# Tongji-MIC-Lab/TDVC

Hardware: AMD Instinct MI355X
Metric: 1080p P-frames/sec (encode + reconstruct, lambda=2048 config) (higher is better)
Workload: dtype f16; 1 GPU; 1x 1920x1080 (padded 1088x1920) 7-frame synthetic GOP (seed 1234), batch 1, P-frames coded in GOP order; gop=7, batch=1, parallelism=gop-sharded x1, weights=closed-form filler (no checkpoint ships)

## Files before the change

### include/tdvc_hip.h

```cpp
#ifndef TDVC_HIP_H
#define TDVC_HIP_H

#include <stdint.h>

#ifdef __cplusplus
extern "C" {
#endif

#define TDVC_OK 0
#define TDVC_EINVAL (-1)
#define TDVC_ENOSUP (-2)

typedef struct {
  void* p;
  int32_t N, H, W, C;
  int64_t sn;
  int32_t sp;
  int32_t dtype;
} tdvc_fmap;

enum { TDVC_F16 = 0, TDVC_F32 = 1 };
enum { TDVC_ACT_NONE = 0, TDVC_ACT_RELU = 1, TDVC_ACT_LRELU = 2, TDVC_ACT_CLAMP01 = 3, TDVC_ACT_SIGMOID = 4 };
enum { TDVC_GDN_NONE = 0, TDVC_GDN_FWD = 1, TDVC_GDN_INV = 2 };
enum { TDVC_OUT_NHWC = 0,
// ... 56 lines not shown
  const float* bias;
  int32_t act1; float slope1;
  int32_t act2; float slope2;
  int32_t add_input;
  tdvc_fmap res2;
} tdvc_conv_pair_desc;
int64_t tdvc_conv_pair_packed_bytes(void);
int tdvc_pack_conv_pair_weights(const float* w1_oihw, const float* w2_oihw, uint16_t* dst);
int tdvc_conv_pair_supported(const tdvc_conv_pair_desc* d);
int tdvc_conv_pair(const tdvc_conv_pair_desc* d, void* stream);

typedef struct {
  tdvc_fmap s, a, y;
  int32_t nslices;
  int32_t slice_stride;
  const void* wt;
  const float* bias_t;
  const void* w3;
  const float* bias3;
  float slope;
} tdvc_lf_tail_desc;
int tdvc_lf_tail_supported(const tdvc_lf_tail_desc* d);
int tdvc_lf_tail(const tdvc_lf_tail_desc* d, void* stream);

typedef struct {
  tdvc_fmap x, om, y;
  const void* w;
  const float* bias;
  int32_t groups;
  int32_t act; float slope; int32_t round_before_act;
  void* x_planar;
} tdvc_dcn_desc;
int tdvc_dcn_fused(const tdvc_dcn_desc* d, void* stream);

int tdvc_dcn_v2_forward_f32(const float* input, const float* weight, const float* bias,
                            const float* offset, const float* mask, float* output,
                            int B, int C, int H, int W, int Cout,
                            int kh, int kw, int sh, int sw, int ph, int pw, int dh, int dw,
                            int deformable_group, void* stream);
int tdvc_dcn_v2_backward_f32(const float* input, const float* weight, const float* bias,
                             const float* offset, const float* mask, const float* grad_output,
                             float* grad_input, float* grad_offset, float* grad_mask,
                             float* grad_weight, float* grad_bias, float* columns,
                             int B, int C, int H, int W, int Cout,
                             int kh, int kw, int sh, int sw, int ph, int pw, int dh, int dw,
                             int deformable_group, void* stream);
// ... 220 lines not shown
```

### tdvc_amd/_lib.py

```python
from __future__ import annotations

import ctypes as C
import os

_HERE = os.path.dirname(os.path.abspath(__file__))
LIB_PATH = os.path.join(_HERE, "libtdvc_hip.so")

MAX_TAPS = 49
F16, F32 = 0, 1
ACT_NONE, ACT_RELU, ACT_LRELU, ACT_CLAMP01, ACT_SIGMOID = 0, 1, 2, 3, 4
GDN_NONE, GDN_FWD, GDN_INV = 0, 1, 2
OUT_NHWC, OUT_SHUFFLE2, OUT_NCHW_F32 = 0, 1, 2


class FMapDesc(C.Structure):
    _fields_ = [("p", C.c_void_p), ("N", C.c_int32), ("H", C.c_int32), ("W", C.c_int32), ("C", C.c_int32),
                ("sn", C.c_int64), ("sp", C.c_int32), ("dtype", C.c_int32)]


class ConvDesc(C.Structure):
    _fields_ = [("x", FMapDesc), ("y", FMapDesc), ("w", C.c_void_p), ("bias", C.c_void_p),
                ("cout", C.c_int32), ("ntaps", C.c_int32),
                ("tap_dy", C.c_int8 * MAX_TAPS), ("tap_dx", C.c_int8 * MAX_TAPS),
                ("kh", C.c_int32), ("kw", C.c_int32), ("stride", C.c_int32), ("pad", C.c_int32),
                ("ck", C.c_int32), ("square_input", C.c_int32), ("gdn", C.c_int32),
                ("aux", FMapDesc), ("act", C.c_int32), ("slope", C.c_float),
                ("round_before_act", C.c_int32), ("res", FMapDesc), ("res2", FMapDesc), ("out_mode", C.c_int32), ("s2d", C.c_int32),
                ("bcast_T", C.c_int32), ("bcast_slope", C.c_float), ("chan_sum", C.c_void_p), ("flow", FMapDesc)]


class DcnDesc(C.Structure):
    _fields_ = [("x", FMapDesc), ("om", FMapDesc), ("y", FMapDesc), ("w", C.c_void_p), ("bias", C.c_void_p),
                ("groups", C.c_int32), ("act", C.c_int32), ("slope", C.c_float), ("round_before_act", C.c_int32), ("x_planar", C.c_void_p)]


class ConvPairDesc(C.Structure):
    _fields_ = [("x", FMapDesc), ("y", FMapDesc), ("w", C.c_void_p), ("bias", C.c_void_p), ("act1", C.c_int32), ("slope1", C.c_float),
                ("act2", C.c_int32), ("slope2", C.c_float), ("add_input", C.c_int32), ("res2", FMapDesc)]


class LfTailDesc(C.Structure):
    _fields_ = [("s", FMapDesc), ("a", FMapDesc), ("y", FMapDesc), ("nslices", C.c_int32), ("slice_stride", C.c_int32),
                ("wt", C.c_void_p), ("bias_t", C.c_void_p), ("w3", C.c_void_p), ("bias3", C.c_void_p), ("slope", C.c_float)]


class WgradReduceJob(C.Structure):
    _fields_ = [("work", C.c_void_p), ("bwork", C.c_void_p), ("row_off", C.c_void_p), ("chan_off", C.c_void_p), ("tap_off", C.c_void_p),
                ("bias_index", C.c_void_p), ("dw", C.c_void_p), ("db", C.c_void_p), ("scale", C.c_float),
                ("nworkers", C.c_int32), ("cow", C.c_int32), ("ciw", C.c_int32), ("ntaps", C.c_int32), ("cout", C.c_int32), ("cin", C.c_int32),
                ("wblocks", C.c_int32), ("nblocks", C.c_int32)]


_P = C.c_void_p
_FM = C.POINTER(FMapDesc)


class CdfTablesDesc(C.Structure):
    _fields_ = [("cdfs", _P), ("sizes", _P), ("offsets", _P), ("stride", C.c_int32), ("ncdfs", C.c_int32)]


class CdfTablesDevDesc(C.Structure):
    _fields_ = [("cdf16", _P), ("starts", _P), ("sizes", _P), ("offsets", _P), ("n16", C.c_int32), ("ncdfs", C.c_int32)]


class ArLoopDesc(C.Structure):
    _fields_ = [("y_hat", FMapDesc), ("params", FMapDesc), ("x1", FMapDesc), ("pc", FMapDesc), ("gp", FMapDesc),
# ... 78 lines not shown
    "tdvc_ssim_level": (_i, [_P, _P, _i, _i, _i, _i, _P, _i, _f, _f, _P, _P, _P, _i64, _P]),
    "tdvc_avgpool2_pad_f32": (_i, [_P, _i64, _i, _i, _P, _P]),
    "tdvc_ssim_level_backward": (_i, [_P, _P, _i, _i, _i, _i, _P, _i, _f, _f, _P, _P, _f, _P, _P, _P]),
    "tdvc_msssim_level_grads": (_i, [_P, _P, _P, _i, _i, _P, _P, _P, _P, _P]),
    "tdvc_dcn_col2im_work_floats": (_i64, [_i, _i, _i, _i]),
    "tdvc_dcn_col2im_tile": (_i, []),
    "tdvc_dcn_col2im": (_i, [_FM, _FM, _FM, _i, _P, _FM, _P, _i64, _P]),
    "tdvc_dcn_col2im_det": (_i, [_FM, _FM, _FM, _i, _P, _FM, _P, _i64, _P, _P, _P, _i, _P]),
    "tdvc_dcn_far_apply": (_i, [_P, _P, _P, _i, _P, _P]),
    "tdvc_conv_wgrad_work_floats": (_i64, [_i] * 6),
    "tdvc_conv_wgrad": (_i, [_FM, _FM] + [_i] * 6 + [_P] * 5 + [_i, _f, _P, _P, _i64, _P]),
    "tdvc_conv_wgrad_bias": (_i, [_FM, _FM] + [_i] * 6 + [_P] * 5 + [_i, _f, _P, _P, _P, _P, _i64, _P]),
    "tdvc_conv_wgrad_partials": (_i, [_FM, _FM] + [_i] * 6 + [_P] * 5 + [_i, _f, _P, _P, _P, _P, _i64, C.POINTER(WgradReduceJob), _P]),
    "tdvc_wgrad_reduce_batch": (_i, [_P, _P, _i, _i, _P]),
    "tdvc_gdn_backward": (_i, [_FM, _FM, _FM, _i, _FM, _FM, _P]),
    "tdvc_mul2_accumulate": (_i, [_FM, _FM, _FM, _P]),
    "tdvc_dcn_fused": (_i, [C.POINTER(DcnDesc), _P]),
    "tdvc_conv_pair_packed_bytes": (_i64, []),
    "tdvc_pack_conv_pair_weights": (_i, [_P, _P, _P]),
    "tdvc_conv_pair_supported": (_i, [C.POINTER(ConvPairDesc)]),
    "tdvc_conv_pair": (_i, [C.POINTER(ConvPairDesc), _P]),
    "tdvc_lf_tail_supported": (_i, [C.POINTER(LfTailDesc)]),
    "tdvc_lf_tail": (_i, [C.POINTER(LfTailDesc), _P]),
    "tdvc_dcn_v2_forward_f32": (_i, [_P] * 6 + [_i] * 14 + [_P]),
    "tdvc_dcn_v2_backward_f32": (_i, [_P] * 12 + [_i] * 14 + [_P]),
    "tdvc_nchw_to_fmap": (_i, [_P, _i, _FM, _P]),
    "tdvc_fmap_to_nchw": (_i, [_FM, _i, _P, _P]),
    "tdvc_scale_act_res": (_i, [_FM, _P, _i, _f, _FM, _f, _FM, _FM, _P]),
    "tdvc_add_flow": (_i, [_FM, _FM, _P]),
    "tdvc_bcast_add_act": (_i, [_FM, _FM, _i, _f, _P]),
    "tdvc_channel_sum": (_i, [_FM, _P, _i, _P]),
    "tdvc_se_gate": (_i, [_P, _i, _f, _i, _i, _i, _P, _P, _P, _P, _P, _P]),
    "tdvc_upsample2x": (_i, [_FM, _FM, _P]),
    "tdvc_avgpool2": (_i, [_FM, _FM, _P]),
    "tdvc_spynet_level_input": (_i, [_FM, _FM, _FM, _FM, _FM, _P]),
    "tdvc_resize_bilinear": (_i, [_FM, _FM, _P, _P]),
    "tdvc_avgpool_k_work_floats": (_i64, [_i, _i, _i, _i, _i]),
    "tdvc_avgpool_k": (_i, [_FM, _i, _P, _i, _i, _P, _i64, _P]),
    "tdvc_patch_match": (_i, [_P, _P, _i, _i, _i, _i, _P, _P]),
    "tdvc_match_gather": (_i, [_FM, _FM, _P, _i, _i, _i, _FM, _P]),
    "tdvc_eb_forward": (_i, [_FM, _P, _FM, _FM, _P, _P, _i, _P]),
    "tdvc_gc_forward": (_i, [_FM, _FM, _FM, _P, _P, _i, _P]),
    "tdvc_quantize": (_i, [_FM, _FM, _FM, _P]),
    "tdvc_rans_encode": (_i64, [_P, _P, _i64, _P, C.c_int32, _P, _P, _P, _i64]),
    "tdvc_rans_decode": (_i, [_P, _i64, _P, _i64, _P, C.c_int32, _P, _P, _P]),
    "tdvc_rans_encode_lanes": (_i64, [_P, _P, _i64, _i, _i, _P, C.c_int32, _P, _P, _P, _i64]),
# ... 40 lines not shown
```

### tdvc_amd/csrc/conv_dispatch.hip

```cpp
#include <stdlib.h>

#include "conv_common.h"

using convk::ConvParams;
bool conv_v2_eligible(const tdvc_conv_desc* d, int Ho, int Wo); int launch_conv_v2(const ConvParams& p, int cout_blocks, int N, hipStream_t st);
bool conv_v3_eligible(const tdvc_conv_desc* d, int Ho, int Wo); int launch_conv_v3(const ConvParams& p, int cout_blocks, int N, hipStream_t st);
bool conv_v5_eligible(const tdvc_conv_desc* d, int Ho, int Wo); int launch_conv_v5(const ConvParams& p, int cout_blocks, int N, hipStream_t st); int conv_v5_chan_sum_rows(int Ho, int Wo, int cout_blocks, int N);
bool conv_v7_eligible(const tdvc_conv_desc* d, const ConvParams& p, int Ho, int Wo); int launch_conv_v7(const ConvParams& p, int cout_blocks, int N, hipStream_t st);
bool conv_v9_eligible(const tdvc_conv_desc* d, int Ho, int Wo, bool v3_ok); int launch_conv_v9(const ConvParams& p, int ck8, int cout_tiles32, int N, hipStream_t st);
bool conv_v10_eligible(const tdvc_conv_desc* d, const ConvParams& p, int Ho, int Wo); int launch_conv_v10(const ConvParams& p, int cout_blocks, int N, hipStream_t st);
bool conv_v11_eligible(const tdvc_conv_desc* d, const ConvParams& p, int Ho, int Wo); int launch_conv_v11(const ConvParams& p, int cout_blocks, int N, hipStream_t st);
int conv_row_geometry(const tdvc_conv_desc* d, const ConvParams& p, int Ho, int Wo); int launch_conv_row(int geo, const ConvParams& p, int N, hipStream_t st);
bool conv_c8_eligible(const tdvc_conv_desc* d, const ConvParams& p, int Ho, int Wo); int launch_conv_c8(const ConvParams& p, int N, hipStream_t st);
bool conv_n16_eligible(const tdvc_conv_desc* d, int Ho, int Wo); int launch_conv_n16(const ConvParams& p, int N, hipStream_t st);
bool gdn128_eligible(const tdvc_conv_desc* d, const ConvParams& p, int Ho, int Wo); int launch_gdn128(const ConvParams& p, int N, hipStream_t st);
int conv_direct_lds_bytes(const tdvc_conv_desc* d);
int conv_cout_tiles(int cout);
int launch_conv_direct(const ConvParams& p, int ck8, int stride, int N, hipStream_t st);
int conv_f32_validate(const tdvc_conv_desc* d, int& Ho, int& Wo);

namespace {
const char* const kSwitchEnv[convk::SW_COUNT] = {nullptr, "TDVC_CONV_NO_V3", "TDVC_CONV_NO_V5", "TDVC_CONV_NO_V7", "TDVC_CONV_NO_V9", "TDVC_CONV_NO_V10",
                                                 "TDVC_CONV_NO_V11", "TDVC_CONV_NO_ROW", "TDVC_CONV_NO_C8", "TDVC_CONV_NO_N16", "TDVC_CONV_NO_GDN128", "TDVC_CONV_NO_HEAD3"};
int g_enabled[convk::SW_COUNT] = {1, 1, 1, 1, 1, 1, 1, 15, 1, 1, 1, 1};
// ... 222 lines not shown
  ConvParams p;
  Pick k = {d, 0, 0, -1};
  if (const int rc = prepare(d, p, k.Ho, k.Wo)) return rc;
  p.reverse = query != LAUNCH ? 0 : next_walk_reverse();
  const Entry* e = select(k, p);
  const bool csum_ok = e && e->name == kNameV5 && k.cout_blocks() == 1 && p.simple == 2;
  if (query_rows) return csum_ok ? conv_v5_chan_sum_rows(k.Ho, k.Wo, 1, k.N()) : 0;
  if (query == QUERY_FLOW) return conv_flow_ok(d, e, p) && (!d->flow.p || flow_map_ok(d, k.Ho, k.Wo)) ? 1 : 0;
  TDVC_CHECK(!d->chan_sum || (csum_ok && (reinterpret_cast<uintptr_t>(d->chan_sum) & 15) == 0),
             "tdvc_conv2d: chan_sum on a conv whose kernel has no fused channel sum (tdvc_conv_chan_sum_rows() == 0) or unaligned");
  p.csum = d->chan_sum;
  if (!e) return TDVC_EINVAL;
  if (d->flow.p) {
    TDVC_CHECK(conv_flow_ok(d, e, p) && flow_map_ok(d, k.Ho, k.Wo), "%s", kFlowMsg);
    p.flow = to_dev(d->flow);
  }
  kernel_name(e, k, g_last_kernel);
  return e->launch(k, p, reinterpret_cast<hipStream_t>(stream));
}

}

void tdvc_conv_walk_advance(int launches) { g_walk_parity += (unsigned)launches; }

extern "C" void tdvc_debug_set_conv_walk(int mode) { g_walk_mode = mode; }
extern "C" int tdvc_conv2d(const tdvc_conv_desc* d, void* stream) { return conv2d_impl(d, stream, LAUNCH); }
extern "C" int tdvc_conv_chan_sum_rows(const tdvc_conv_desc* d) { return conv2d_impl(d, nullptr, QUERY_ROWS); }
extern "C" int tdvc_conv_flow_supported(const tdvc_conv_desc* d) { return conv2d_impl(d, nullptr, QUERY_FLOW); }
extern "C" const char* tdvc_last_conv_kernel(void) { return g_last_kernel; }

extern "C" const char* tdvc_conv_select(const tdvc_conv_desc* d) {
  static thread_local char name[48];
  if (!d) { tdvc_set_error("tdvc_conv_select: null descriptor"); return nullptr; }
  if (d->x.dtype == TDVC_F32) {
    int Ho, Wo;
    if (d->flow.p) { tdvc_set_error("%s", kFlowMsg); return nullptr; }
    return conv_f32_validate(d, Ho, Wo) == TDVC_OK ? "conv_f32" : nullptr;
  }
  ConvParams p;
  Pick k = {d, 0, 0, -1};
  if (prepare(d, p, k.Ho, k.Wo) != TDVC_OK) return nullptr;
  const Entry* e = select(k, p);
  if (!e) return nullptr;
  if (d->flow.p && !(conv_flow_ok(d, e, p) && flow_map_ok(d, k.Ho, k.Wo))) { tdvc_set_error("%s", kFlowMsg); return nullptr; }
  kernel_name(e, k, name);
  return name;
// ... 2 lines not shown
```

### tdvc_amd/csrc/lib.cpp

```cpp
#include <hip/hip_runtime.h>
#include <stdarg.h>
#include <stddef.h>
#include <stdio.h>

#include <mutex>

#include "../../include/tdvc_hip.h"

static thread_local char g_err[512] = "";

void tdvc_set_error(const char* fmt, ...) {
  va_list ap;
  va_start(ap, fmt);
  vsnprintf(g_err, sizeof(g_err), fmt, ap);
  va_end(ap);
}

static_assert(sizeof(tdvc_cdf_tables) == 32 && offsetof(tdvc_cdf_tables, ncdfs) == 28, "tdvc_cdf_tables layout");
static_assert(sizeof(tdvc_cdf_tables_dev) == 40 && offsetof(tdvc_cdf_tables_dev, ncdfs) == 36, "tdvc_cdf_tables_dev layout");
static_assert(sizeof(tdvc_ar_loop) == 272 && offsetof(tdvc_ar_loop, sym_dev) == 264, "tdvc_ar_loop layout");
static_assert(sizeof(tdvc_lf_tail_desc) == 168 && offsetof(tdvc_lf_tail_desc, slope) == 160, "tdvc_lf_tail_desc layout");
static_assert(sizeof(tdvc_lanes_enc) == 104 && offsetof(tdvc_lanes_enc, info) == 96, "tdvc_lanes_enc layout");

extern "C" int tdvc_abi_version(void) { return 16; }
extern "C" const char* tdvc_last_error(void) { return g_err; }

static thread_local const int* g_pred = nullptr;
static thread_local int g_pred_taken = 0, g_pred_last = 0;
static thread_local const int* g_pred_img = nullptr;
static thread_local int g_pred_img_n = 0;

extern "C" int tdvc_set_predicate(const int* flag) {
  if (reinterpret_cast<uintptr_t>(flag) & 3) { tdvc_set_error("tdvc_set_predicate: flag must be 4-byte aligned"); return TDVC_EINVAL; }
  if (flag && g_pred_img) { tdvc_set_error("tdvc_set_predicate: a per-image predicate is set (clear it first)"); return TDVC_EINVAL; }
  g_pred = flag;
  return TDVC_OK;
}
extern "C" int tdvc_set_predicate_images(const int* flags, int n) {
  if (!flags || n == 0) { g_pred_img = nullptr; g_pred_img_n = 0; return TDVC_OK; }
  if (reinterpret_cast<uintptr_t>(flags) & 3) { tdvc_set_error("tdvc_set_predicate_images: flags must be 4-byte aligned"); return TDVC_EINVAL; }
  if (n < 1 || n > TDVC_MAX_PREDICATE_IMAGES) { tdvc_set_error("tdvc_set_predicate_images: 1 <= n <= %d images, got %d", TDVC_MAX_PREDICATE_IMAGES, n); return TDVC_EINVAL; }
  if (g_pred) { tdvc_set_error("tdvc_set_predicate_images: a launch predicate is set (clear it first)"); return TDVC_EINVAL; }
  g_pred_img = flags; g_pred_img_n = n;
  return TDVC_OK;
}
const int* tdvc_launch_predicate_images(int N) {
  if (!g_pred_img || N != g_pred_img_n) return nullptr;
// ... 52 lines not shown
```

### tdvc_amd/csrc/pointwise.hip

```cpp
#include "pointwise_common.h"

namespace {

__global__ void nchw_to_fmap_kernel(const float* src, int C, FMap y) {
  const long npix = (long)y.H * y.W;
  const long i = (long)blockIdx.x * blockDim.x + threadIdx.x;
  if (i >= npix * y.N) return;
  const int n = (int)(i / npix);
  const long pix = i % npix;
  for (int c0 = 0; c0 < y.C; c0 += 8) {
    float v[8];
#pragma unroll
    for (int j = 0; j < 8; ++j) v[j] = (c0 + j < C) ? src[((long)n * C + c0 + j) * npix + pix] : 0.f;
    store8(y, n, pix, c0, v);
  }
}

__global__ void fmap_to_nchw_kernel(FMap x, int C, float* dst) {
  const long npix = (long)x.H * x.W;
  const long i = (long)blockIdx.x * blockDim.x + threadIdx.x;
  if (i >= npix * x.N) return;
  const int n = (int)(i / npix);
  const long pix = i % npix;
  for (int c0 = 0; c0 < C; c0 += 8) {
// ... 242 lines not shown
  if (tid < Cmid) {
    float s = b1[tid];
    for (int c = 0; c < C; ++c) s += w1[tid * C + c] * mean[c];
    mid[tid] = s > 0.f ? s : 0.f;
  }
  __syncthreads();
  if (tid < C) {
    float s = b2[tid];
    for (int j = 0; j < Cmid; ++j) s += w2[tid * Cmid + j] * mid[j];
    gate[(long)n * C + tid] = 1.f / (1.f + expf(-s));
  }
}

__global__ void upsample2x_kernel(FMap x, FMap y) {
  const int chunks = x.C / 8;
  const long npix = (long)y.H * y.W;
  const long i = (long)blockIdx.x * blockDim.x + threadIdx.x;
  if (i >= npix * chunks * y.N) return;
  const int c = (int)(i % chunks) * 8;
  const long t = i / chunks;
  const long pix = t % npix;
  const int n = (int)(t / npix);
  const int oy = (int)(pix / y.W), ox = (int)(pix % y.W);
  const float sy = fmaxf((oy + 0.5f) * 0.5f - 0.5f, 0.f), sx = fmaxf((ox + 0.5f) * 0.5f - 0.5f, 0.f);
  const int y0 = (int)sy, x0 = (int)sx;
  const int y1 = y0 + (y0 < x.H - 1), x1 = x0 + (x0 < x.W - 1);
  const float ly1 = sy - y0, lx1 = sx - x0, ly0 = 1.f - ly1, lx0 = 1.f - lx1;
  float a[8], b[8], cc[8], d[8], v[8];
  load8(x, n, (long)y0 * x.W + x0, c, a);
  load8(x, n, (long)y0 * x.W + x1, c, b);
  load8(x, n, (long)y1 * x.W + x0, c, cc);
  load8(x, n, (long)y1 * x.W + x1, c, d);
#pragma unroll
  for (int j = 0; j < 8; ++j) v[j] = ly0 * (lx0 * a[j] + lx1 * b[j]) + ly1 * (lx0 * cc[j] + lx1 * d[j]);
  store8(y, n, pix, c, v);
}

__global__ void avgpool2_kernel(FMap x, FMap y) {
  const long npix = (long)y.H * y.W;
  const long i = (long)blockIdx.x * blockDim.x + threadIdx.x;
  if (i >= npix * y.N) return;
  const int n = (int)(i / npix);
  const long pix = i % npix;
  const int oy = (int)(pix / y.W), ox = (int)(pix % y.W);
  const float* xp = reinterpret_cast<const float*>(x.p) + (long)n * x.sn;
  float* yp = reinterpret_cast<float*>(y.p) + (long)n * y.sn + pix * y.sp;
  const long p00 = ((long)(2 * oy) * x.W + 2 * ox) * x.sp, p10 = p00 + (long)x.W * x.sp;
  for (int c = 0; c < y.C; ++c)
    yp[c] = (xp[p00 + c] + xp[p00 + x.sp + c] + xp[p10 + c] + xp[p10 + x.sp + c]) * 0.25f;
}

struct PyramidMaps { FMap x[2]; FMap y[2][5]; };
template <bool VEC>
__global__ __launch_bounds__(256) void avgpool2_pyramid_kernel(const PyramidMaps a) {
  __shared__ __attribute__((aligned(16))) float lv[2][16 * 16 * 4];
  const int m = blockIdx.z & 1, n = blockIdx.z >> 1, tid = threadIdx.x;
  const int C = a.y[0][0].C;
// ... 691 lines not shown
```

### tdvc_amd/model/modules.py

```python
from __future__ import annotations

import torch
import torch.nn as nn

from .. import ops
from ..ops import ACT_LRELU, ACT_NONE, ACT_RELU, FM
from .ring import SlotRing


class PackCache:

    def _pk(self, key, fn):
        c = self.__dict__.setdefault("_packed", {})
        if key not in c:
            c[key] = fn()
        return c[key]


def _dev(m: nn.Module):
    return next(m.parameters()).device


def pk_conv(owner: PackCache, name: str, conv: nn.Module, **kw) -> ops.PackedConv:
    def build():
# ... 58 lines not shown
        if self.conv1.in_channels == 64 and ops.conv_pair_supported(x, out, res2) and (out is None or out.desc().p != x.desc().p):
            pp = self._pk("pair", lambda: ops.pack_conv_pair(self.conv1.weight, self.conv1.bias, self.conv2.weight, self.conv2.bias))
            return ops.conv_pair(x, pp, out=out, act1=ACT_RELU, act2=ACT_NONE, add_input=True, res2=res2)
        t = ops.conv(x, pk_conv(self, "c1", self.conv1), act=ACT_RELU)
        return ops.conv(t, pk_conv(self, "c2", self.conv2), out=out, res=x, res2=res2)


def res_stack(n, ch=64):
    return nn.Sequential(*[Res_Block(ch) for _ in range(n)])


def run_stack(stack, x: FM, out: FM | None = None, res2: FM | None = None) -> FM:
    n = len(stack)
    for i, blk in enumerate(stack):
        last = i == n - 1
        x = blk.run(x, out=out if last else None, res2=res2 if last else None)
    return x


PYRAMID_FUSED = True
FLOW_EPILOGUE = True
RESID_FUSED = True
RGB_HEAD = True


def glue_fusions_allowed(module: nn.Module, traced: bool = False) -> bool:
    return not module.training and ops.TAPE is None and ops.PROFILE is None and not traced


class SPyNetBasicModule(nn.Module):
    def __init__(self):
        super().__init__()
        ch = [8, 32, 64, 32, 16, 2]
        self.basic_module = nn.Sequential(*[ConvAct(ch[i], ch[i + 1], 7, 1, 3) for i in range(5)])


class SPyNet(nn.Module, PackCache):

    def __init__(self):
        super().__init__()
        self.basic_module = nn.ModuleList([SPyNetBasicModule() for _ in range(6)])
        self.register_buffer("mean", torch.tensor([0.485, 0.456, 0.406]).view(1, 3, 1, 1))
        self.register_buffer("std", torch.tensor([0.229, 0.224, 0.225]).view(1, 3, 1, 1))

    def compute_flow(self, ref: FM, supp: FM, fused: bool = False, f32: bool = False) -> FM:
        if fused and PYRAMID_FUSED and ops.avgpool2_pyramid_supported(ref, supp):
# ... 83 lines not shown
            t = ops.conv(cat2.ch(64 * k, 64), pk_conv(self, "l3_1", self.conv_l3_1), **lr)
            ops.conv(t, pk_conv(self, "l3_2", self.conv_l3_2), out=cat3.ch(64 * k, 64), **lr)
        cats = {1: cat1, 2: cat2, 3: cat3}
        up_o1 = None
        off = None
        for i in (3, 2, 1):
            lv = f"l{i}"
            c = cats[i]
            if i == 1 and fuse and FLOW_EPILOGUE:
                flow = self.spynet.run(cur32, ref32, fused=fuse)
            o1 = ops.conv(c, pk_conv(self, "c11" + lv, self.offset_conv11[lv]), **lr)
            if i == 3:
                if ops.conv_pair_supported(o1):
                    c1_, c2_ = self.offset_conv11_1[lv], self.offset_conv12[lv]
                    pp = self._pk("pair_l3", lambda: ops.pack_conv_pair(c1_.weight, c1_.bias, c2_.weight, c2_.bias))
                    off = ops.conv_pair(o1, pp, act1=ACT_LRELU, slope1=0.1, act2=ACT_LRELU, slope2=0.1, add_input=False)
                else:
                    o1 = ops.conv(o1, pk_conv(self, "c11_1" + lv, self.offset_conv11_1[lv]), **lr)
                    off = ops.conv(o1, pk_conv(self, "c12" + lv, self.offset_conv12[lv]), **lr)
            else:
                ops.conv(o1, pk_conv(self, "c11_1" + lv, self.offset_conv11_1[lv]), out=up_o1.ch(64, 64), **lr)
                off = ops.conv(up_o1, pk_conv(self, "ff" + lv, self.feat_fusion[lv]), flow=flow if i == 1 else None, **lr)
            if i > 1:
                up = ops.upsample2x(off)
                up_o1 = FM.empty(B, up.H, up.W, 128, dtype=adt, device=dev)
                ops.conv(up, pk_conv(self, "upc", self.upsample_conv), out=up_o1.ch(0, 64))
        if flow is None:
            flow = self.spynet.run(cur32, ref32, fused=fuse, f32=f32)
            if ops.TAPE is not None:
                off = ops.clone(off)
            ops.add_flow(off, flow)
        sums = []
        e = ops.conv(off, pk_conv(self, "ff_", self.feat_fusion_), chan_sum=sums)
        return self.attn.run(e, sums=sums)


class DCN(nn.Module, PackCache):

    def __init__(self, cin, cout, k, stride, padding, dilation=1, deformable_groups=1):
        super().__init__()
        assert k == 3 and stride == 1 and padding == 1 and dilation == 1
        self.deformable_groups = deformable_groups
        self.weight = nn.Parameter(torch.zeros(cout, cin, k, k))
        self.bias = nn.Parameter(torch.zeros(cout))
        self.conv_offset_mask = nn.Conv2d(cin, deformable_groups * 3 * k * k, k, stride, padding)

    def run(self, x: FM, y: FM, out: FM, act=ACT_NONE, slope=0.0) -> FM:
        om = ops.conv(y, pk_conv(self, "om", self.conv_offset_mask))
        pc = self._pk("w", lambda: ops.pack_conv(self.weight, self.bias, stride=1, pad=1, ck=8 * self.deformable_groups,
# ... 324 lines not shown
```

### tdvc_amd/ops.py

```python
from __future__ import annotations

import ctypes as C
from dataclasses import dataclass

import numpy as np
import torch

from . import _lib as L
from . import convpack
from ._lib import (ACT_CLAMP01, ACT_LRELU, ACT_NONE, ACT_RELU, GDN_FWD, GDN_INV, GDN_NONE, OUT_NCHW_F32,
                   OUT_NHWC, OUT_SHUFFLE2)


_raw_stream = torch._C._cuda_getCurrentRawStream
_cur_dev = torch._C._cuda_getDevice
FORCE_STREAM = None
FORCE_KEEP = None


def _stream():
    if FORCE_STREAM is not None:
        return C.c_void_p(FORCE_STREAM)
    return C.c_void_p(_raw_stream(_cur_dev()))

# ... 429 lines not shown
    if nchw_out is not None:
        assert nchw_out.shape == (x.N, pc.cout, Ho, Wo) and nchw_out.dtype == torch.float32 and nchw_out.is_contiguous()
        d.out_mode = OUT_NCHW_F32
        d.y = L.FMapDesc(nchw_out.data_ptr(), x.N, Ho, Wo, pc.cout, pc.cout * Ho * Wo, 1, L.F32)
        ret = nchw_out
    else:
        if pc.shuffle:
            d.out_mode = OUT_SHUFFLE2
            if out is None:
                out = FM.empty(x.N, 2 * Ho, 2 * Wo, pad8(pc.cout // 4), dtype=out_dtype, device=x.t.device)
        else:
            d.out_mode = OUT_NHWC
            if out is None:
                out = FM.empty(x.N, Ho, Wo, pc.cout if (out_dtype == torch.float32 and not x.f32) else pad8(pc.cout),
                               dtype=out_dtype, device=x.t.device)
        d.y = out.desc()
        ret = out
    return d, ret, Ho, Wo, pc, rec_pc


def conv(x: FM, pc: PackedConv, out: FM | None = None, act=ACT_NONE, slope=0.0, res: FM | None = None,
         res2: FM | None = None, gdn=GDN_NONE, aux: FM | None = None, square=False, out_dtype=None,
         round16=False, nchw_out: torch.Tensor | None = None, bcast_T=0, bcast_slope=0.0, chan_sum: list | None = None,
         flow: FM | None = None) -> FM | torch.Tensor:
    d, ret, Ho, Wo, pc, rec_pc = conv_desc(x, pc, out, act, slope, res, res2, gdn, aux, square, out_dtype, round16, nchw_out, bcast_T, bcast_slope)
    if chan_sum is not None and TAPE is None and FUSE_CHAN_SUM:
        rows = L.lib().tdvc_conv_chan_sum_rows(C.byref(d))
        if rows > 0:
            part = torch.empty((x.N, rows, pc.cout), dtype=torch.float32, device=x.t.device)
            d.chan_sum = part.data_ptr()
            chan_sum.append((part, rows))
    if bcast_T and TAPE is not None and not _IN_BACKWARD:
        raise L.TdvcHipError("conv: bcast_T is an inference-only fusion (under the tape use conv + bcast_add_act)")
    if flow is not None:
        if (TAPE is not None and not _IN_BACKWARD) or chan_sum is not None or nchw_out is not None:
            raise L.TdvcHipError("conv: flow is an inference-only fusion of an fmap output, not combined with chan_sum (use conv + add_flow)")
        d.flow = flow.desc()
        if L.lib().tdvc_conv_flow_supported(C.byref(d)) != 1:
            d.flow = _NULL_FM
            L.check(L.lib().tdvc_conv2d(C.byref(d), _stream()), "conv2d")
            _log_predicated()
            add_flow(ret, flow)
            return ret
    if PROFILE is not None:
        e0, e1 = torch.cuda.Event(enable_timing=True), torch.cuda.Event(enable_timing=True)
        e0.record()
        L.check(L.lib().tdvc_conv2d(C.byref(d), _stream()), "conv2d")
        e1.record()
        PROFILE.append(dict(kernel=L.lib().tdvc_last_conv_kernel().decode(),
                            shape=f"{pc.kh}x{pc.kw} s{pc.stride} {x.C}->{pc.cout} @{x.H}x{x.W}" + (" f32out" if out_dtype == torch.float32 else "") + (" nchw" if nchw_out is not None else ""),
                            e0=e0, e1=e1,
                            flops=2.0 * x.N * Ho * Wo * pc.cout * x.C * len(pc.taps),
                            flops_real=(x.N * Ho * Wo * pc.flops_per_px) if pc.s2d else 2.0 * x.N * Ho * Wo * pc.cout * pc.cin_real * len(pc.taps),
                            bytes=2.0 * x.N * (x.H * x.W * x.C + Ho * Wo * pc.cout * (4 if pc.shuffle else 1) / (4 if pc.shuffle else 1))))
        _rec("conv", x, rec_pc, None if nchw_out is not None else ret, act, slope, res, res2, gdn, aux, square, nchw_out)
        return ret
    L.check(L.lib().tdvc_conv2d(C.byref(d), _stream()), "conv2d")
    _log_predicated()
    _rec("conv", x, rec_pc, None if nchw_out is not None else ret, act, slope, res, res2, gdn, aux, square, nchw_out)
    return ret


class rgb_head_kernel:

    def __init__(self, enable: bool):
        self.enable = bool(enable)

    def __enter__(self):
        if not self.enable:
            L.lib().tdvc_debug_enable_conv_head3(0)
        return self

    def __exit__(self, *exc):
        if not self.enable:
            L.lib().tdvc_debug_enable_conv_head3(1)
        return False


class PackedConvPair:

    def __init__(self, w: torch.Tensor, bias: torch.Tensor):
        self.w, self.bias = w, bias

# ... 1021 lines not shown
```

Measured before the change: 52.68 frames/s.

## Fuse bilinear 2x upsample into the following 3x3 conv for offset path

Adds a dedicated HIP kernel that computes the bilinear 2x upsample of a 64-channel low-resolution map inside LDS and feeds it directly into a 3x3 64->64 MFMA convolution. A ring of low-resolution rows is streamed in by loader waves while the other waves store outputs. This removes the materialised full-resolution upsampled intermediate and its global write and read-back in the offset pyramid. The cost is a large, complex kernel with its own row pipelining and a fallback when conditions aren't met; the bilinear math is factored into a shared header.

```diff
diff --git a/include/tdvc_hip.h b/include/tdvc_hip.h
--- a/include/tdvc_hip.h
+++ b/include/tdvc_hip.h
@@ -102,6 +102,15 @@
 } tdvc_lf_tail_desc;
 int tdvc_lf_tail_supported(const tdvc_lf_tail_desc* d);
 int tdvc_lf_tail(const tdvc_lf_tail_desc* d, void* stream);
+
+typedef struct {
+  tdvc_fmap x;
+  tdvc_fmap y;
+  const void* w;
+  const float* bias;
+} tdvc_conv_up2x_desc;
+int tdvc_conv_up2x_supported(const tdvc_conv_up2x_desc* d);
+int tdvc_conv_up2x(const tdvc_conv_up2x_desc* d, void* stream);
 
 typedef struct {
   tdvc_fmap x, om, y;
diff --git a/tdvc_amd/_lib.py b/tdvc_amd/_lib.py
--- a/tdvc_amd/_lib.py
+++ b/tdvc_amd/_lib.py
@@ -42,6 +42,10 @@
 class LfTailDesc(C.Structure):
     _fields_ = [("s", FMapDesc), ("a", FMapDesc), ("y", FMapDesc), ("nslices", C.c_int32), ("slice_stride", C.c_int32),
                 ("wt", C.c_void_p), ("bias_t", C.c_void_p), ("w3", C.c_void_p), ("bias3", C.c_void_p), ("slope", C.c_float)]
+
+
+class ConvUp2xDesc(C.Structure):
+    _fields_ = [("x", FMapDesc), ("y", FMapDesc), ("w", C.c_void_p), ("bias", C.c_void_p)]
 
 
 class WgradReduceJob(C.Structure):
@@ -166,6 +170,8 @@
     "tdvc_conv_pair": (_i, [C.POINTER(ConvPairDesc), _P]),
     "tdvc_lf_tail_supported": (_i, [C.POINTER(LfTailDesc)]),
     "tdvc_lf_tail": (_i, [C.POINTER(LfTailDesc), _P]),
+    "tdvc_conv_up2x_supported": (_i, [C.POINTER(ConvUp2xDesc)]),
+    "tdvc_conv_up2x": (_i, [C.POINTER(ConvUp2xDesc), _P]),
     "tdvc_dcn_v2_forward_f32": (_i, [_P] * 6 + [_i] * 14 + [_P]),
     "tdvc_dcn_v2_backward_f32": (_i, [_P] * 12 + [_i] * 14 + [_P]),
     "tdvc_nchw_to_fmap": (_i, [_P, _i, _FM, _P]),
diff --git a/tdvc_amd/csrc/conv_dispatch.hip b/tdvc_amd/csrc/conv_dispatch.hip
--- a/tdvc_amd/csrc/conv_dispatch.hip
+++ b/tdvc_amd/csrc/conv_dispatch.hip
@@ -268,6 +268,7 @@
 }
 
 void tdvc_conv_walk_advance(int launches) { g_walk_parity += (unsigned)launches; }
+int tdvc_conv_walk_take() { return next_walk_reverse(); }
 
 extern "C" void tdvc_debug_set_conv_walk(int mode) { g_walk_mode = mode; }
 extern "C" int tdvc_conv2d(const tdvc_conv_desc* d, void* stream) { return conv2d_impl(d, stream, LAUNCH); }
diff --git a/tdvc_amd/csrc/lib.cpp b/tdvc_amd/csrc/lib.cpp
--- a/tdvc_amd/csrc/lib.cpp
+++ b/tdvc_amd/csrc/lib.cpp
@@ -22,7 +22,9 @@
 static_assert(sizeof(tdvc_lf_tail_desc) == 168 && offsetof(tdvc_lf_tail_desc, slope) == 160, "tdvc_lf_tail_desc layout");
 static_assert(sizeof(tdvc_lanes_enc) == 104 && offsetof(tdvc_lanes_enc, info) == 96, "tdvc_lanes_enc layout");
 
-extern "C" int tdvc_abi_version(void) { return 16; }
+static_assert(sizeof(tdvc_conv_up2x_desc) == 96 && offsetof(tdvc_conv_up2x_desc, y) == 40 && offsetof(tdvc_conv_up2x_desc, bias) == 88, "tdvc_conv_up2x_desc layout");
+
+extern "C" int tdvc_abi_version(void) { return 17; }
 extern "C" const char* tdvc_last_error(void) { return g_err; }
 
 static thread_local const int* g_pred = nullptr;
diff --git a/tdvc_amd/csrc/og_fused.hip b/tdvc_amd/csrc/og_fused.hip
--- /dev/null
+++ b/tdvc_amd/csrc/og_fused.hip
@@ -0,0 +1,349 @@
+#include <string.h>
+
+#include <type_traits>
+
+#include "conv_dma.h"
+#include "upsample2x.h"
+
+using convk::glds16;
+using convk::raw_barrier;
+
+int tdvc_conv_walk_take();
+
+namespace {
+
+constexpr int UP_SW = 64, UP_RPX = UP_SW + 2, UP_PXB = 128, UP_ROWB = 9 * 1024;
+constexpr int UP_LPX = UP_SW / 2 + 2, UP_LROWB = 5 * 1024, UP_LRING = 6;
+constexpr int UP_D = 3;
+constexpr int UP_SROW = 8192;
+constexpr int UP_H0 = 0, UP_L0 = UP_H0 + 4 * UP_ROWB, UP_S0 = UP_L0 + UP_LRING * UP_LROWB, UP_B0 = UP_S0 + 4 * UP_SROW, UP_LDS = UP_B0 + 256;
+constexpr int UP_NTHR = 512;
+static_assert(UP_RPX * UP_PXB <= UP_ROWB && UP_LPX * UP_PXB <= UP_LROWB, "ring rows");
+static_assert(UP_D >= 3 && UP_LRING > UP_D + 1 && UP_D + 2 <= UP_LRING, "low ring conditions");
+static_assert((UP_L0 % 1024) == 0 && (UP_S0 % 16) == 0 && UP_LDS <= 160 * 1024, "LDS");
+
+struct Up2xParams {
+  const half_t* x; long x_sn; int x_sp;
+  half_t* y; long y_sn; int y_sp;
+  const half_t* w;
+  const float* bias;
+  const half_t* zeros;
+  half_t* dump;
+  int N, H, W;
+  int Hl, Wl;
+  int strips;
+  int reverse;
+};
+
+__device__ __forceinline__ int up_f(int q) { return (q >> 1) & 7; }
+__device__ __forceinline__ int up_sigma(int r) { return r < 4 ? 2 * r : (r >= 12 ? 2 * r - 16 : 2 * r - 7); }
+__device__ __forceinline__ int up_g(int q) { return (q >> 1) & 7; }
+
+__global__ __launch_bounds__(UP_NTHR, 1) void conv_up2x_kernel(const Up2xParams p) {
+  extern __shared__ __attribute__((aligned(1024))) unsigned char smem[];
+  const unsigned lds0 = static_cast<unsigned>(reinterpret_cast<uintptr_t>(smem));
+  const int tid = threadIdx.x, lane = tid & 63;
+  const int wave = __builtin_amdgcn_readfirstlane(tid >> 6);
+  const bool loader = wave < 4;
+  const int wq = wave & 3;
+  const int cg = wave & 3, cbp = wave >> 2;
+  const int r16 = lane & 15, kb = lane >> 4;
+
+  const int nwg = (int)gridDim.x, b = (int)blockIdx.x;
+  int pos_slot = b;
+  if ((nwg & 7) == 0) pos_slot = (b & 7) * (nwg >> 3) + (b >> 3);
+  if (p.reverse) pos_slot = nwg - 1 - pos_slot;
+  const long allrows = (long)p.N * p.strips * p.H;
+  const long run_begin = (allrows * pos_slot / nwg) & ~1L, run_end = (allrows * (pos_slot + 1) / nwg) & ~1L;
+
+  half8 wf[18];
+  {
+    const int co = 16 * cg + r16;
+    const half_t* wb = p.w + ((long)(co >> 5) * 2 * 18 * 64 + (kb & 1) * 32 + (co & 31)) * 8 + (long)(kb >> 1) * 512;
+#pragma unroll
+    for (int tap = 0; tap < 9; ++tap)
+#pragma unroll
+      for (int kc = 0; kc < 2; ++kc) wf[tap * 2 + kc] = *reinterpret_cast<const half8*>(wb + ((long)kc * 18 + tap * 2) * 512);
+#pragma unroll
+    for (int i = 0; i < 18; ++i) asm volatile("" : "+v"(wf[i]));
+  }
+  if (tid < 64) reinterpret_cast<float*>(smem + UP_B0)[tid] = p.bias[tid];
+  const int boff = UP_B0 + (16 * cg + 4 * kb) * 4;
+
+  int foff[3];
+#pragma unroll
+  for (int dx = 0; dx < 3; ++dx) {
+    const int q = 32 * cbp + dx + up_sigma(r16);
+    foff[dx] = q * UP_PXB + ((kb ^ up_f(q)) << 4);
+  }
+  int doff[2];
+#pragma unroll
+  for (int cb = 0; cb < 2; ++cb) {
+    const int q = 32 * cbp + 16 * cb + up_sigma(r16), c = 2 * cg + (kb >> 1);
+    doff[cb] = q * UP_PXB + ((c ^ up_g(q)) << 4) + 8 * (kb & 1);
+  }
+  const int u_s = tid & 7;
+  const int u_q[2] = {tid >> 3, (tid >> 3) + 2};
+  int u_w[2];
+#pragma unroll
+  for (int j = 0; j < 2; ++j) u_w[j] = u_q[j] * UP_PXB + ((u_s ^ up_f(u_q[j])) << 4);
+  const bool u_second = tid >= UP_NTHR - 16;
+
+  auto run = [&](auto LOADERc) __attribute__((always_inline)) {
+  constexpr bool LOADER = decltype(LOADERc)::value;
+  const int d_px[2] = {8 * wq + (lane >> 3), 32 + (lane >> 3)};
+  int soff[2];
+#pragma unroll
+  for (int j = 0; j < 2; ++j) soff[j] = d_px[j] * p.x_sp + (lane & 7) * 8;
+  const int s_t = tid & 255;
+  int s_px[2], s_co[2];
+#pragma unroll
+  for (int j = 0; j < 2; ++j) {
+    const int it = s_t + 256 * j;
+    s_px[j] = it >> 3;
+    s_co[j] = ((it & 7) ^ up_g(it >> 3)) << 3;
+  }
+
+  f32x4 acc[3][2];
+
+  for (long pos = run_begin; pos < run_end;) {
+    const int sid = (int)(pos / p.H);
+    const int ra = (int)(pos - (long)sid * p.H), rb = (int)min((long)p.H, ra + (run_end - pos));
+    const int rows = rb - ra;
+    pos += rows;
+    const int n = sid / p.strips, strip = sid - n * p.strips;
+    const int c0 = strip * UP_SW;
+    const int lc0 = (c0 >> 1) - 1;
+    const int i_last = min(rb, p.H - 1);
+
+    unsigned lok = 0;
+#pragma unroll
+    for (int j = 0; j < 2; ++j) {
+      const int col = lc0 + d_px[j];
+      lok |= (d_px[j] < UP_LPX && col >= 0 && col < p.Wl) ? (1u << j) : 0u;
+    }
+    bool s_ok[2];
+    int y_lo[2];
+#pragma unroll
+    for (int j = 0; j < 2; ++j) {
+      const int col = c0 + s_px[j];
+      s_ok[j] = col < p.W;
+      y_lo[j] = col * p.y_sp + s_co[j];
+    }
+    Up2xTap u_tx[2];
+    bool u_ok[2];
+    int u_a[2], u_b[2];
+#pragma unroll
+    for (int j = 0; j < 2; ++j) {
+      const int col = c0 - 1 + u_q[j];
+      u_ok[j] = col >= 0 && col < p.W;
+      u_tx[j] = up2x_tap(min(max(col, 0), p.W - 1), p.Wl);
+      u_a[j] = (u_tx[j].i0 - lc0) * UP_PXB + u_s * 16;
+      u_b[j] = (u_tx[j].i1 - lc0) * UP_PXB + u_s * 16;
+    }
+    half_t* const yimg = p.y + (long)n * p.y_sn;
+    const long yrow_stride = (long)p.W * p.y_sp, xrow_stride = (long)p.Wl * p.x_sp;
+    const half_t* const xcol = p.x + (long)n * p.x_sn + (long)lc0 * p.x_sp;
+#pragma unroll
+    for (int s3 = 0; s3 < 3; ++s3)
+#pragma unroll
+      for (int cb = 0; cb < 2; ++cb) acc[s3][cb] = f32x4{0.f, 0.f, 0.f, 0.f};
+
+    auto low_top = [&](int kk) __attribute__((always_inline)) -> int {
+      return up2x_tap(min(max(ra - 1 + kk, 0), i_last), p.Hl).i1;
+    };
+    auto issue_low = [&](int l) __attribute__((always_inline)) -> int {
+      const half_t* base = xcol + l * xrow_stride;
+      const unsigned dst = lds0 + UP_L0 + (__builtin_amdgcn_readfirstlane(l) % UP_LRING) * UP_LROWB;
+      glds16((lok & 1u) ? base + soff[0] : p.zeros, dst + wq * 1024);
+      if (wq == 0) {
+        glds16((lok & 2u) ? base + soff[1] : p.zeros, dst + 4 * 1024);
+        return 2;
+      }
+      return 1;
+    };
+    auto land_wait = [&](int cnt) __attribute__((always_inline)) {
+      if (cnt >= 4) asm volatile("s_waitcnt vmcnt(4)" ::: "memory");
+      else if (cnt >= 2) asm volatile("s_waitcnt vmcnt(2)" ::: "memory");
+      else if (cnt == 1) asm volatile("s_waitcnt vmcnt(1)" ::: "memory");
+      else asm volatile("s_waitcnt vmcnt(0)" ::: "memory");
+    };
+    auto phase_u = [&](int jj) __attribute__((always_inline)) {
+      const int iA = ra - 1 + 2 * jj, iB = iA + 1;
+      const bool okA = iA >= 0 && iA < p.H, okB = iB < p.H;
+      const Up2xTap tyA = up2x_tap(min(max(iA, 0), p.H - 1), p.Hl), tyB = up2x_tap(min(iB, p.H - 1), p.Hl);
+      const int r0 = okA ? tyA.i0 : tyB.i0, r1 = okA ? tyA.i1 : tyB.i1;
+      const unsigned char* l0 = smem + UP_L0 + (__builtin_amdgcn_readfirstlane(r0) % UP_LRING) * UP_LROWB;
+      const unsigned char* l1 = smem + UP_L0 + (__builtin_amdgcn_readfirstlane(r1) % UP_LRING) * UP_LROWB;
+      unsigned char* hA = smem + UP_H0 + ((2 * jj) & 3) * UP_ROWB;
+      unsigned char* hB = hA + UP_ROWB;
+      auto item = [&](int j) __attribute__((always_inline)) {
+        const half8 a = *reinterpret_cast<const half8*>(l0 + u_a[j]), bq = *reinterpret_cast<const half8*>(l0 + u_b[j]);
+        const half8 c = *reinterpret_cast<const half8*>(l1 + u_a[j]), d = *reinterpret_cast<const half8*>(l1 + u_b[j]);
+        const bool wA = okA && u_ok[j], wB = okB && u_ok[j];
+        half8 oA, oB;
+#pragma unroll
+        for (int e = 0; e < 8; ++e) {
+          const float fa = (float)a[e], fb_ = (float)bq[e], fc = (float)c[e], fd = (float)d[e];
+          const float vA = up2x_mix(tyA, u_tx[j], fa, fb_, fc, fd), vB = up2x_mix(tyB, u_tx[j], fa, fb_, fc, fd);
+          oA[e] = wA ? (half_t)vA : (half_t)0.f;
+          oB[e] = wB ? (half_t)vB : (half_t)0.f;
+        }
+        *reinterpret_cast<half8*>(hA + u_w[j]) = oA;
+        *reinterpret_cast<half8*>(hB + u_w[j]) = oB;
+      };
+      item(0);
+      if (!LOADER && u_second) item(1);
+    };
+
+    const int jlast = rows >> 1;
+    int nxt = up2x_tap(max(ra - 1, 0), p.Hl).i0;
+    if constexpr (LOADER) {
+      const int top = low_top(2 * min(UP_D, jlast) + 1);
+      for (; nxt <= top; ++nxt) issue_low(nxt);
+    }
+    asm volatile("s_waitcnt vmcnt(0)" ::: "memory");
+    raw_barrier();
+    phase_u(0);
+    raw_barrier();
+
+    const int J = jlast + 2;
+    int n1 = 0;
+    auto step = [&](auto PHc, int j) __attribute__((always_inline)) {
+      constexpr int PH0 = decltype(PHc)::value;
+      if constexpr (!LOADER) {
+#pragma unroll
+        for (int r = 0; r < 2; ++r) {
+          const int srow = ra + 2 * j - 4 + r;
+          if (srow >= ra && srow < rb) {
+            const unsigned char* sb = smem + UP_S0 + ((2 * j - 2 + r) & 3) * UP_SROW;
+            half_t* const yrow = yimg + srow * yrow_stride;
+#pragma unroll
+            for (int i = 0; i < 2; ++i) {
+              const half8 yv = *reinterpret_cast<const half8*>(sb + (s_t + 256 * i) * 16);
+              *reinterpret_cast<half8*>(s_ok[i] ? yrow + y_lo[i] : p.dump + (s_t + 256 * i) * 8) = yv;
+            }
+          }
+        }
+        if (j + 1 <= jlast) phase_u(j + 1);
+      }
+      if (j <= jlast) {
+        const f32x4 bias4 = *reinterpret_cast<const f32x4*>(smem + boff);
+#pragma unroll
+        for (int r = 0; r < 2; ++r) {
+          const int PH = (PH0 + r) % 3;
+          const int SD = (PH + 1) % 3;
+          const int k = 2 * j + r;
+          const unsigned char* xb = smem + UP_H0 + (k & 3) * UP_ROWB;
+          half8 fb[3][2];
+          auto load_group = [&](int gi, int buf) __attribute__((always_inline)) {
+            const int kc = gi / 3, dx = gi - 3 * kc;
+            const unsigned char* b0 = xb + (foff[dx] ^ (kc << 6));
+#pragma unroll
+            for (int cb = 0; cb < 2; ++cb) fb[buf][cb] = *reinterpret_cast<const half8*>(b0 + cb * 16 * UP_PXB);
+          };
+          load_group(0, 0);
+          load_group(1, 1);
+#pragma unroll
+          for (int gi = 0; gi < 6; ++gi) {
+            const int kc = gi / 3, dx = gi - 3 * kc;
+            if (gi + 2 < 6) load_group(gi + 2, (gi + 2) % 3);
+#pragma unroll
+            for (int dyo = 0; dyo < 3; ++dyo) {
+              const int dy = 2 - dyo;
+              const int slot = (PH + 3 - dy) % 3;
+#pragma unroll
+              for (int cb = 0; cb < 2; ++cb) {
+                const bool first = dy == 0 && gi == 0;
+                acc[slot][cb] = __builtin_amdgcn_mfma_f32_16x16x32_f16(wf[(dy * 3 + dx) * 2 + kc], fb[gi % 3][cb], first ? bias4 : acc[slot][cb], 0, 0, 0);
+              }
+            }
+          }
+          unsigned char* sb = smem + UP_S0 + (k & 3) * UP_SROW;
+#pragma unroll
+          for (int cb = 0; cb < 2; ++cb) {
+            const f32x4 v = acc[SD][cb];
+            const half4 h = {(half_t)v[0], (half_t)v[1], (half_t)v[2], (half_t)v[3]};
+            *reinterpret_cast<half4*>(sb + doff[cb]) = h;
+          }
+        }
+      }
+      if constexpr (LOADER) {
+        if (j + 1 <= jlast) phase_u(j + 1);
+        int n0 = 0;
+        if (j + 1 + UP_D <= jlast && nxt <= low_top(2 * (j + 1 + UP_D) + 1)) n0 = issue_low(nxt++);
+        land_wait(n0 + n1);
+        n1 = n0;
+      }
+      raw_barrier();
+    };
+    for (int j = 0; j < J; j += 3) {
+      step(std::integral_constant<int, 0>{}, j);
+      if (j + 1 < J) step(std::integral_constant<int, 2>{}, j + 1);
+      if (j + 2 < J) step(std::integral_constant<int, 1>{}, j + 2);
+    }
+  }
+  };
+  if (loader) run(std::true_type{});
+  else run(std::false_type{});
+}
+
+bool up_disjoint(const tdvc_fmap& x, const tdvc_fmap& y) {
+  const uintptr_t xa = (uintptr_t)x.p, ya = (uintptr_t)y.p;
+  const uintptr_t xe = xa + 2 * ((uintptr_t)(x.N - 1) * x.sn + ((uintptr_t)x.H * x.W - 1) * x.sp + x.C);
+  const uintptr_t ye = ya + 2 * ((uintptr_t)(y.N - 1) * y.sn + ((uintptr_t)y.H * y.W - 1) * y.sp + y.C);
+  return !(xa < ye && ya < xe);
+}
+
+const char* up_refusal(const tdvc_conv_up2x_desc* d) {
+  if (!d) return "null descriptor";
+  const tdvc_fmap &x = d->x, &y = d->y;
+  if (x.dtype != TDVC_F16 || y.dtype != TDVC_F16) return "x and y must be fp16 maps";
+  if (!fmap_ok16(x) || !fmap_ok16(y)) return "x and y must be 16-byte aligned maps with channels and strides in multiples of 8";
+  if (x.C != 64 || y.C != 64) return "x and y must have 64 channels";
+  if (y.N != x.N || y.H != 2 * x.H || y.W != 2 * x.W) return "y must have x's batch and twice its rows and columns";
+  if ((long)y.H * y.W < convk::LARGE_MAP_PIXELS || y.H < 16) return "the output is under the floor (8192 pixels, 16 rows)";
+  if ((long)y.H * y.W * y.sp >= (1L << 31) || (long)x.H * x.W * x.sp >= (1L << 31)) return "element offsets within an image must fit 32 bits";
+  if (!d->w || !d->bias || !aligned16(d->w) || !aligned16(d->bias)) return "weights / bias missing or misaligned";
+  if (!up_disjoint(x, y)) return "y overlaps x (the kernel is out of place)";
+  tdvc_conv_desc c;
+  memset(&c, 0, sizeof(c));
+  c.x = y;
+  c.x.p = x.p; c.x.sp = 64; c.x.sn = (int64_t)y.H * y.W * 64;
+  c.y = y;
+  c.w = d->w; c.bias = d->bias;
+  c.cout = 64; c.ntaps = 9; c.kh = c.kw = 3; c.stride = 1; c.pad = 1; c.ck = 32;
+  for (int t = 0; t < 9; ++t) { c.tap_dy[t] = (int8_t)(t / 3); c.tap_dx[t] = (int8_t)(t % 3); }
+  c.act = TDVC_ACT_NONE; c.out_mode = TDVC_OUT_NHWC;
+  const char* k = tdvc_conv_select(&c);
+  if (!k || strcmp(k, "conv_row") != 0) return "tdvc_conv2d would not run the 3x3 conv on conv_row";
+  return nullptr;
+}
+
+}
+
+extern "C" int tdvc_conv_up2x_supported(const tdvc_conv_up2x_desc* d) { return up_refusal(d) ? 0 : 1; }
+
+extern "C" int tdvc_conv_up2x(const tdvc_conv_up2x_desc* d, void* stream) {
+  if (const char* why = up_refusal(d)) {
+    tdvc_set_error("tdvc_conv_up2x: %s", why);
+    return TDVC_EINVAL;
+  }
+  const void* zeros = nullptr;
+  void* dump = nullptr;
+  if (const int zrc = tdvc_scratch_pages(&zeros, &dump)) return zrc;
+  Up2xParams q;
+  q.x = reinterpret_cast<const half_t*>(d->x.p); q.x_sn = d->x.sn; q.x_sp = d->x.sp;
+  q.y = reinterpret_cast<half_t*>(d->y.p); q.y_sn = d->y.sn; q.y_sp = d->y.sp;
+  q.w = reinterpret_cast<const half_t*>(d->w);
+  q.bias = d->bias;
+  q.zeros = reinterpret_cast<const half_t*>(zeros);
+  q.dump = reinterpret_cast<half_t*>(dump);
+  q.N = d->y.N; q.H = d->y.H; q.W = d->y.W;
+  q.Hl = d->x.H; q.Wl = d->x.W;
+  q.strips = (q.W + UP_SW - 1) / UP_SW;
+  q.reverse = tdvc_conv_walk_take();
+  const long allrows = (long)q.N * q.strips * q.H;
+  const int grid = allrows / 2 < 256 ? (int)(allrows / 2) : 256;
+  return convk::launch_big_lds<&conv_up2x_kernel>("tdvc_conv_up2x", UP_LDS, dim3(grid), dim3(UP_NTHR), UP_LDS, reinterpret_cast<hipStream_t>(stream), q);
+}
diff --git a/tdvc_amd/csrc/pointwise.hip b/tdvc_amd/csrc/pointwise.hip
--- a/tdvc_amd/csrc/pointwise.hip
+++ b/tdvc_amd/csrc/pointwise.hip
@@ -1,4 +1,5 @@
 #include "pointwise_common.h"
+#include "upsample2x.h"
 
 namespace {
 
@@ -288,17 +289,14 @@
   const long pix = t % npix;
   const int n = (int)(t / npix);
   const int oy = (int)(pix / y.W), ox = (int)(pix % y.W);
-  const float sy = fmaxf((oy + 0.5f) * 0.5f - 0.5f, 0.f), sx = fmaxf((ox + 0.5f) * 0.5f - 0.5f, 0.f);
-  const int y0 = (int)sy, x0 = (int)sx;
-  const int y1 = y0 + (y0 < x.H - 1), x1 = x0 + (x0 < x.W - 1);
-  const float ly1 = sy - y0, lx1 = sx - x0, ly0 = 1.f - ly1, lx0 = 1.f - lx1;
+  const Up2xTap ty = up2x_tap(oy, x.H), tx = up2x_tap(ox, x.W);
   float a[8], b[8], cc[8], d[8], v[8];
-  load8(x, n, (long)y0 * x.W + x0, c, a);
-  load8(x, n, (long)y0 * x.W + x1, c, b);
-  load8(x, n, (long)y1 * x.W + x0, c, cc);
-  load8(x, n, (long)y1 * x.W + x1, c, d);
-#pragma unroll
-  for (int j = 0; j < 8; ++j) v[j] = ly0 * (lx0 * a[j] + lx1 * b[j]) + ly1 * (lx0 * cc[j] + lx1 * d[j]);
+  load8(x, n, (long)ty.i0 * x.W + tx.i0, c, a);
+  load8(x, n, (long)ty.i0 * x.W + tx.i1, c, b);
+  load8(x, n, (long)ty.i1 * x.W + tx.i0, c, cc);
+  load8(x, n, (long)ty.i1 * x.W + tx.i1, c, d);
+#pragma unroll
+  for (int j = 0; j < 8; ++j) v[j] = up2x_mix(ty, tx, a[j], b[j], cc[j], d[j]);
   store8(y, n, pix, c, v);
 }
 
diff --git a/tdvc_amd/csrc/upsample2x.h b/tdvc_amd/csrc/upsample2x.h
--- /dev/null
+++ b/tdvc_amd/csrc/upsample2x.h
@@ -0,0 +1,17 @@
+#pragma once
+
+namespace {
+
+struct Up2xTap { int i0, i1; float w0, w1; };
+__device__ __forceinline__ Up2xTap up2x_tap(int o, int n) {
+  const float s = fmaxf((o + 0.5f) * 0.5f - 0.5f, 0.f);
+  const int i0 = (int)s;
+  const int i1 = i0 + (i0 < n - 1);
+  const float w1 = s - i0, w0 = 1.f - w1;
+  return {i0, i1, w0, w1};
+}
+__device__ __forceinline__ float up2x_mix(const Up2xTap& ty, const Up2xTap& tx, float a, float b, float c, float d) {
+  return ty.w0 * (tx.w0 * a + tx.w1 * b) + ty.w1 * (tx.w0 * c + tx.w1 * d);
+}
+
+}
diff --git a/tdvc_amd/model/modules.py b/tdvc_amd/model/modules.py
--- a/tdvc_amd/model/modules.py
+++ b/tdvc_amd/model/modules.py
@@ -104,6 +104,7 @@
 FLOW_EPILOGUE = True
 RESID_FUSED = True
 RGB_HEAD = True
+OFFSET_UP_FUSED = True
 
 
 def glue_fusions_allowed(module: nn.Module, traced: bool = False) -> bool:
@@ -233,9 +234,12 @@
                 ops.conv(o1, pk_conv(self, "c11_1" + lv, self.offset_conv11_1[lv]), out=up_o1.ch(64, 64), **lr)
                 off = ops.conv(up_o1, pk_conv(self, "ff" + lv, self.feat_fusion[lv]), flow=flow if i == 1 else None, **lr)
             if i > 1:
-                up = ops.upsample2x(off)
-                up_o1 = FM.empty(B, up.H, up.W, 128, dtype=adt, device=dev)
-                ops.conv(up, pk_conv(self, "upc", self.upsample_conv), out=up_o1.ch(0, 64))
+                up_o1 = FM.empty(B, 2 * off.H, 2 * off.W, 128, dtype=adt, device=dev)
+                if fuse and OFFSET_UP_FUSED:
+                    ops.conv(off, pk_conv(self, "upc", self.upsample_conv), out=up_o1.ch(0, 64), up2x=True)
+                else:
+                    up = ops.upsample2x(off)
+                    ops.conv(up, pk_conv(self, "upc", self.upsample_conv), out=up_o1.ch(0, 64))
         if flow is None:
             flow = self.spynet.run(cur32, ref32, fused=fuse, f32=f32)
             if ops.TAPE is not None:
diff --git a/tdvc_amd/ops.py b/tdvc_amd/ops.py
--- a/tdvc_amd/ops.py
+++ b/tdvc_amd/ops.py
@@ -475,7 +475,16 @@
 def conv(x: FM, pc: PackedConv, out: FM | None = None, act=ACT_NONE, slope=0.0, res: FM | None = None,
          res2: FM | None = None, gdn=GDN_NONE, aux: FM | None = None, square=False, out_dtype=None,
          round16=False, nchw_out: torch.Tensor | None = None, bcast_T=0, bcast_slope=0.0, chan_sum: list | None = None,
-         flow: FM | None = None) -> FM | torch.Tensor:
+         flow: FM | None = None, up2x: bool = False) -> FM | torch.Tensor:
+    if up2x:
+        plain = (act == ACT_NONE and res is None and res2 is None and gdn == GDN_NONE and aux is None and not square and not round16
+                 and nchw_out is None and not bcast_T and chan_sum is None and flow is None and out_dtype in (None, torch.float16))
+        if plain and TAPE is None and PROFILE is None:
+            ret = _conv_up2x(x, pc, out)
+            if ret is not None:
+                return ret
+        return conv(upsample2x(x), pc, out, act, slope, res, res2, gdn, aux, square, out_dtype, round16, nchw_out, bcast_T, bcast_slope,
+                    chan_sum, flow)
     d, ret, Ho, Wo, pc, rec_pc = conv_desc(x, pc, out, act, slope, res, res2, gdn, aux, square, out_dtype, round16, nchw_out, bcast_T, bcast_slope)
     if chan_sum is not None and TAPE is None and FUSE_CHAN_SUM:
         rows = L.lib().tdvc_conv_chan_sum_rows(C.byref(d))
@@ -512,6 +521,27 @@
     _log_predicated()
     _rec("conv", x, rec_pc, None if nchw_out is not None else ret, act, slope, res, res2, gdn, aux, square, nchw_out)
     return ret
+
+
+def _conv_up2x(x: FM, pc: PackedConv, out: FM | None) -> FM | None:
+    if x.f32 or (pc.cin, pc.cout, pc.kh, pc.kw, pc.ck, pc.stride, pc.pad) != (64, 64, 3, 3, 32, 1, 1) or pc.s2d or pc.shuffle:
+        return None
+    if [tuple(t) for t in pc.taps] != [(dy, dx) for dy in range(3) for dx in range(3)]:
+        return None
+    if out is not None and (out.f32 or (out.N, out.H, out.W, out.C) != (x.N, 2 * x.H, 2 * x.W, 64)):
+        return None
+    d = L.ConvUp2xDesc()
+    d.x = x.desc()
+    d.y = out.desc() if out is not None else L.FMapDesc(16, x.N, 2 * x.H, 2 * x.W, 64, 4 * x.H * x.W * 64, 64, L.F16)
+    d.w, d.bias = pc.w.data_ptr(), pc.bias.data_ptr()
+    if not L.lib().tdvc_conv_up2x_supported(C.byref(d)):
+        return None
+    if out is None:
+        out = FM.empty(x.N, 2 * x.H, 2 * x.W, 64, device=x.t.device)
+        d.y = out.desc()
+    L.check(L.lib().tdvc_conv_up2x(C.byref(d), _stream()), "conv_up2x")
+    _log_predicated()
+    return out
 
 
 class rgb_head_kernel:
```

Measured after the change: 53.03 frames/s, median of 6. Within noise of the previous version (+0.7%).
